# c-white/blacklight

Hardware: AMD Instinct MI355X
Metric: Mrays/sec + achieved HBM GB/s, 1024^2 camera over 256^3 GRMHD grid (higher is better)
Workload: dtype f64

## Files before the change

blacklight_amd/csrc/bl_geodesic.hip:

```cpp
#include "bl_kernel_util.h"
#include "bl_geodesic_common.h"
#include "bl_distance_closed.h"

namespace {

struct RayState {
  double y[8];
  double kt;
};

template <bool kWithDistance, bool kSpinZero>
__device__ __forceinline__ void rhs(const BlSpacetime &st, const double y[8], double kt, double k[8], double *r, int distance = BL_DISTANCE_EXACT) {
  double pos[3] = {y[1], y[2], y[3]};
  double kcov[4] = {kt, y[4], y[5], y[6]};
  double dpos[4], dk[3], ds = 0.0;
  bl_geodesic_rhs<kWithDistance, kSpinZero>(st, pos, kcov, dpos, dk, &ds, r, distance);
  k[0] = dpos[0];
  k[1] = dpos[1];
  k[2] = dpos[2];
  k[3] = dpos[3];
  k[4] = dk[0];
  k[5] = dk[1];
  k[6] = dk[2];
  k[7] = ds;
}

__device__ __forceinline__ long long traversal_to_ray(long long q, int res, const int *tile_order) {
  if (res <= 0) return q;
  int tiles_per_row = res >> 3;
  long long tile = tile_order != nullptr ? (long long)tile_order[q >> 6] : (q >> 6);
  int within = (int)(q & 63);
  long long tile_row = tile / tiles_per_row;
  int tile_col = (int)(tile % tiles_per_row);
  long long m2 = tile_row * 8 + (within >> 3);
  int m1 = tile_col * 8 + (within & 7);
  return m2 * res + m1;
}

__device__ __forceinline__ unsigned long long xcd_traversal(int r, long long j) {
  return (unsigned long long)(((j / BL_XCD_RUN) * BL_XCD_QUEUES + r) * BL_XCD_RUN + j % BL_XCD_RUN);
}
__device__ __forceinline__ long long xcd_queue_rays(int chunk_rays, int r) {
  const long long round = (long long)BL_XCD_RUN * BL_XCD_QUEUES;
  const long long full = chunk_rays / round, rest = chunk_rays - full * round - (long long)r * BL_XCD_RUN;
  return full * BL_XCD_RUN + (rest < 0 ? 0 : (rest < BL_XCD_RUN ? rest : BL_XCD_RUN));
}

}

template <bool kDormandPrince, bool kSpinZero>
__device__ __forceinline__ void bl_start_ray(const BlTraceArgs &P, const BlSpacetime &st, const BlCameraDevice &cam, long long pixel, long long ray, long long q) {
  double u_ind, v_ind, position[4], direction[4], factor;
  bl_pixel_indices(cam, pixel, P.block_locs, &u_ind, &v_ind);
  bl_pixel_ray(st, cam, u_ind, v_ind, position, direction, &factor);
  P.ray_constants[q] = make_double2(direction[0], factor);
  P.ray_out_index[q] = ray;
  if (P.camera_pos != nullptr)
    for (int mu = 0; mu < 4; mu++) P.camera_pos[4 * ray + mu] = position[mu];
  if (P.camera_dir != nullptr)
    for (int mu = 0; mu < 4; mu++) P.camera_dir[4 * ray + mu] = direction[mu];
  double *start = P.ray_start + q;
  const long long stride = P.ray_start_stride;
  RayState s;
  s.y[0] = position[0];
  s.y[1] = position[1];
  s.y[2] = position[2];
  s.y[3] = position[3];
  s.kt = direction[0];
  s.y[4] = direction[1];
  s.y[5] = direction[2];
  s.y[6] = direction[3];
  s.y[7] = 0.0;
  for (int p = 0; p < 7; p++) start[p * stride] = s.y[p];
  start[7 * stride] = s.kt;
  start[8 * stride] = bl_radial_coordinate<kSpinZero>(st, s.y[1], s.y[2], s.y[3]);
  if (kDormandPrince) {
    double k0[8], r_unused;
    rhs<true, kSpinZero>(st, s.y, s.kt, k0, &r_unused);
    for (int p = 0; p < 8; p++) start[(9 + p) * stride] = k0[p];
  }
}

template <bool kDormandPrince, bool kSpinZero>
__global__ void __launch_bounds__(256) bl_ray_init_kernel(BlTraceArgs P) {
  const long long q = (long long)blockIdx.x * blockDim.x + threadIdx.x;
  if (q >= (long long)P.chunk_rays) return;
  const BlSpacetime st = P.st;
  const long long ray = traversal_to_ray(P.chunk_begin + q, P.swizzle_tiles, P.tile_order);
  const long long pixel = P.pixel_map != nullptr ? (long long)P.pixel_map[ray] : ray;
  if (P.cameras == nullptr) {
    bl_start_ray<kDormandPrince, kSpinZero>(P, st, P.cam, pixel, ray, q);
    return;
  }
  const int camera = (int)(pixel / P.pixels_per_camera);
  const long long within = pixel - (long long)camera * P.pixels_per_camera;
  const int first = __builtin_amdgcn_readfirstlane(camera);
  if (__all(camera == first)) {
    const BlCameraDevice cam = P.cameras[first];
    bl_start_ray<kDormandPrince, kSpinZero>(P, st, cam, within, ray, q);
  } else {
    const BlCameraDevice cam = P.cameras[camera];
    bl_start_ray<kDormandPrince, kSpinZero>(P, st, cam, within, ray, q);
  }
}

#ifndef BL_GEO_WAVES
#define BL_GEO_WAVES 2
#endif
#ifndef BL_GEO_ONE_WAVE
#define BL_GEO_ONE_WAVE(integrator, with_time, spin_zero) ((integrator) == BL_INTEGRATOR_DP && ((with_time) || !(spin_zero)))
#endif
__device__ __forceinline__ int lane_here() {
  int l;
  asm volatile("v_mbcnt_lo_u32_b32 %0, -1, 0\n\tv_mbcnt_hi_u32_b32 %0, -1, %0" : "=v"(l));
  return l;
}
__device__ __forceinline__ int opaque_uniform(int v) {
  asm volatile("" : "+s"(v));
  return v;
}
__device__ __forceinline__ double opaque_uniform(double v) {
  asm volatile("" : "+s"(v));
  return v;
}
template <int kIntegrator, bool kTime, bool kSpinZero, bool kShell = false>
__global__ void __launch_bounds__(64, BL_GEO_ONE_WAVE(kIntegrator, kTime, kSpinZero) ? 1 : BL_GEO_WAVES) bl_geodesic_kernel(BlTraceArgs P) {
  const BlSpacetime st = P.st;

  bool have_ray = false;
  bool exhausted = false;
  RayState s;
  double k0[8];
  double h_new = 0.0, r_cur = 0.0, r_prev_sample = 0.0;
  int num_retry = 0, sample_num = 0, trunc_at = -1;
  int skipped = 0;
  int seg = 0;
  unsigned int slot = 0;
  bool previous_fail = false, flag = false;
  for (int p = 0; p < 8; p++) {
    s.y[p] = 0.0;
    k0[p] = 0.0;
  }
  s.kt = 0.0;
  long long block_next = 0, block_end = 0;
  constexpr bool kPark = kIntegrator == BL_INTEGRATOR_DP && !kTime && !kShell;
  __shared__ long long park_lds[5];
  typedef volatile __attribute__((address_space(3))) long long *ParkWord;
  const ParkWord park_word = (ParkWord)park_lds;
  if (kPark && lane_here() == 0) {
    park_lds[0] = reinterpret_cast<long long>(P.parked);
    park_lds[1] = (long long)P.park_capacity;
    const int below = (P.parked == nullptr || P.split_b_hi > 0.0) ? -1 : (P.park_always != 0 ? 64 : (P.park_below < 63 ? P.park_below : 63));
// ... 26 lines not shown
        const unsigned long long per_ray = (unsigned long long)P.ray_max_steps;
        const unsigned long long want = (unsigned long long)count * per_ray;
        const long long over = (long long)(atomicAdd(&P.counters[BL_CNT_COMMITTED], want) + want) - P.record_gate;
        long long refused = over > 0 ? (over + (long long)per_ray - 1) / (long long)per_ray : 0;
        refused = refused < (long long)count ? refused : (long long)count;
        admitted = count - (int)refused;
        long long give_back = -(refused * (long long)per_ray) + ((refused > 0 && over < kGateClosed / 2) ? kGateClosed : 0);
        if (admitted > 0 && P.xcd_state == nullptr) {
          base = atomicAdd(&P.counters[BL_CNT_NEXT_RAY], (unsigned long long)admitted);
          long long beyond = (long long)(base + (unsigned long long)admitted) - (long long)P.chunk_rays;
          beyond = beyond < 0 ? 0 : (beyond < (long long)admitted ? beyond : (long long)admitted);
          give_back -= beyond * (long long)per_ray;
        } else if (admitted > 0) {
          const int own = xcd_here();
          long long got = 0;
          for (int t = xcd_lds[0]; t < BL_XCD_QUEUES && got == 0; t++) {
            const int r = (own + t) & (BL_XCD_QUEUES - 1);
            const long long n_r = xcd_queue_rays(P.chunk_rays, r);
            const long long b = n_r > 0 ? (long long)atomicAdd(&P.xcd_state[r], (unsigned long long)admitted) : 0;
            if (b < n_r) {
              got = n_r - b < (long long)admitted ? n_r - b : (long long)admitted;
              base = (unsigned long long)b | ((unsigned long long)got << 40) | ((unsigned long long)r << 48);
            } else {
              xcd_lds[0] = t + 1;
            }
          }
          give_back -= ((long long)admitted - got) * (long long)per_ray;
        }
        if (give_back != 0) atomicAdd(&P.counters[BL_CNT_COMMITTED], (unsigned long long)give_back);
      }
      base = ((unsigned long long)(unsigned int)__builtin_amdgcn_readlane((int)(base >> 32), leader) << 32)
          | (unsigned long long)(unsigned int)__builtin_amdgcn_readlane((int)base, leader);
      admitted = __builtin_amdgcn_readlane(admitted, leader);
      if (need) {
        const int rank = __popcll(need_mask & ((1ull << lane) - 1ull));
        unsigned long long q = base + (unsigned long long)rank;
        bool wait = false;
        if (P.xcd_state != nullptr) {
          const int got = (int)((base >> 40) & 0xffull);
          q = xcd_traversal((int)(base >> 48), (long long)(base & 0xffffffffffull) + rank);
          wait = rank < admitted && rank >= got && got > 0;
          q = rank < got ? q : ~0ull;
        }
        if (wait) {
        } else if (rank >= admitted || q >= (unsigned long long)P.chunk_rays) {
          exhausted = true;
        } else {
          have_ray = true;
          slot = (unsigned int)q;
          const double *start = P.ray_start + q;
          const long long stride = P.ray_start_stride;
#pragma unroll
          for (int p = 0; p < 7; p++) s.y[p] = start[p * stride];
          s.y[7] = 0.0;
          s.kt = start[7 * stride];
          r_cur = start[8 * stride];
          if (kPark && r_cur < 0.0) {
            have_ray = false;
            atomicAdd(&P.counters[BL_CNT_COMMITTED], (unsigned long long)(-(long long)P.ray_max_steps));
          }
          if (kIntegrator == BL_INTEGRATOR_DP) {
#pragma unroll
            for (int p = 0; p < 8; p++) k0[p] = start[(9 + p) * stride];
          }
          h_new = -P.ray_step * r_cur;
          num_retry = 0;
          previous_fail = false;
          flag = false;
          sample_num = 0;
          skipped = 0;
          seg = 0;
          trunc_at = -1;
          r_prev_sample = 0.0;
        }
      }
    }
    if (kPark) {
      const long long word = park_word[2];
      const int park_below = __builtin_amdgcn_readfirstlane((int)word), park_after = __builtin_amdgcn_readfirstlane((int)(word >> 32));
      const unsigned long long holding = __ballot(have_ray);
      bool park = park_below >= 64;
      if (park_below >= 0 && !park) {
        const long long seen = park_word[3];
        int passes = __builtin_amdgcn_readfirstlane((int)seen);
        const int before = __builtin_amdgcn_readfirstlane((int)(seen >> 32));
        bool dry = passes > 0 || __ballot(exhausted) != 0ull;
        if (!dry && (before & 15) == 15)
          dry = __hip_atomic_load(&P.counters[BL_CNT_NEXT_RAY], __ATOMIC_RELAXED, __HIP_MEMORY_SCOPE_AGENT) >= (unsigned long long)P.chunk_rays;
        dry = __builtin_amdgcn_readfirstlane(dry ? 1 : 0) != 0;
        park_word[3] = dry ? (long long)(((unsigned long long)(unsigned int)before << 32) | (unsigned int)(passes + 1))
                           : (long long)((unsigned long long)(unsigned int)(before + 1) << 32);
        const int quiet = need_mask != 0ull ? 0 : __builtin_amdgcn_readfirstlane((int)park_word[4]) + 1;
        park_word[4] = (long long)quiet;
        park = dry && (__popcll(holding) <= park_below || passes >= park_after || quiet >= P.park_quiet);
      }
      if (park && holding != 0ull) {
        double *const parked = reinterpret_cast<double *>(park_word[0]);
        const long long park_capacity = park_word[1];
        const bool old_ray = have_ray && sample_num >= P.park_age;
        const unsigned long long old_mask = __ballot(old_ray), young_mask = holding & ~old_mask;
        const int leader = __ffsll((long long)holding) - 1;
        const int lane = lane_here();
        unsigned long long base_old = 0ull, base_young = 0ull;
        if (lane == leader) {
          if (old_mask != 0ull) base_old = atomicAdd(&P.counters[BL_CNT_PARKED], (unsigned long long)__popcll(old_mask));
          if (young_mask != 0ull) base_young = atomicAdd(&P.counters[BL_CNT_PARKED_YOUNG], (unsigned long long)__popcll(young_mask));
        }
        const int old_first = __builtin_amdgcn_readlane((int)base_old, leader), young_first = __builtin_amdgcn_readlane((int)base_young, leader);
        const unsigned long long below = (1ull << lane) - 1ull;
        const long long at = old_ray ? (long long)old_first + __popcll(old_mask & below)
                                     : park_capacity - 1 - ((long long)young_first + __popcll(young_mask & below));
        if (have_ray && at >= 0 && at < park_capacity) {
          double *pk = parked + at * BL_PARK_DOUBLES;
#pragma unroll
          for (int p = 0; p < 8; p++) {
            pk[p] = s.y[p];
            pk[8 + p] = k0[p];
          }
          pk[16] = s.kt;
          pk[17] = h_new;
          pk[18] = r_cur;
          pk[19] = r_prev_sample;
          pk[20] = __longlong_as_double((long long)(((unsigned long long)(unsigned int)sample_num << 32) | (unsigned long long)slot));
          pk[21] = __longlong_as_double((long long)(((unsigned long long)(unsigned int)trunc_at << 32) | (unsigned long long)(unsigned int)num_retry));
          pk[22] = __longlong_as_double((long long)(((unsigned long long)((previous_fail ? 1u : 0u) | (flag ? 2u : 0u)) << 32) | (unsigned long long)(unsigned int)seg));
          P.ray_offset[slot] = (long long)atomicAdd(&P.counters[BL_CNT_SAMPLES], (unsigned long long)P.ray_max_steps);
          have_ray = false;
        }
      }
    }
    if (__ballot(have_ray) == 0ull) {
      retire_record_slots(P.records_hot, P.record_stride, block_next, block_end, lane_here());
      break;
    }
#ifdef BL_GEO_STATS
    st_iter += 1;
    st_busy += have_ray ? 1 : 0;
    st_attempt += (have_ray && (kIntegrator != BL_INTEGRATOR_DP || num_retry <= P.ray_max_retries)) ? 1 : 0;
#endif

    int emit = 0;
    int num_steps = 0;
    int num_steps_ideal = 1;
    bool accepted = false;
    bool finish = false;
    double h = 0.0;
    double y5[8], k6[8], y4m[8];
    double rv0[8], rv1[8], rv2[8], rv3[8];
    double r_new = 0.0;
    for (int p = 0; p < 8; p++) {
      y5[p] = 0.0; k6[p] = 0.0; y4m[p] = 0.0; rv0[p] = 0.0; rv1[p] = 0.0; rv2[p] = 0.0; rv3[p] = 0.0;
    }

    if (have_ray) {
      if (kIntegrator == BL_INTEGRATOR_DP) {
        if (num_retry > P.ray_max_retries) {
          flag = true;
          finish = true;
        } else {
          h = h_new;
          double k1[8], k2[8], k3[8], k4[8], k5[8];
          double yt[8], r_stage;
          double t5 = s.y[0], t4 = s.y[0], s5 = s.y[7];
#ifdef BL_DISTANCE_FORCED
          const bool closed = BL_DISTANCE_FORCED != 0;
#else
          const bool closed = P.distance_mode != 0;
#endif
          double s_abs = 0.0, r_low = r_cur;
          if (closed) s5 = 0.0;
#define BL_FOLD(Q, K)                     \
          t5 += kB5[Q] * h * K[0];        \
          t4 += kB4[Q] * h * K[0];        \
          if (!closed) {                  \
            s5 += kB5[Q] * h * K[7];      \
          } else if (kB5[Q] != 0.0) {     \
            const double term = kB5[Q] * h * K[7]; \
            s5 += term;                   \
            s_abs += blm_abs(term);       \
          }
          BL_FOLD(0, k0)
#define BL_STAGE(S, KOUT, ...)                                                  \
          {                                                                      \
            const double *kq[6] = {__VA_ARGS__};                                 \
            _Pragma("unroll") for (int p = 1; p < 7; p++) {                      \
              double acc = s.y[p];                                               \
              _Pragma("unroll") for (int q = 0; q < S; q++) acc += kA[S][q] * h * kq[q][p]; \
              yt[p] = acc;                                                       \
            }                                                                    \
            yt[0] = 0.0; yt[7] = 0.0;                                            \
            rhs<true, kSpinZero>(st, yt, s.kt, KOUT, &r_stage, !closed ? BL_DISTANCE_EXACT : (S == 1 ? BL_DISTANCE_NONE : BL_DISTANCE_CLOSED)); \
            if (closed) r_low = std_min(r_low, r_stage);                         \
            BL_FOLD(S, KOUT)                                                     \
          }
          BL_STAGE(1, k1, k0, k0, k0, k0, k0, k0)
          BL_STAGE(2, k2, k0, k1, k0, k0, k0, k0)
          BL_STAGE(3, k3, k0, k1, k2, k0, k0, k0)
          BL_STAGE(4, k4, k0, k1, k2, k3, k0, k0)
          BL_STAGE(5, k5, k0, k1, k2, k3, k4, k0)
          BL_STAGE(6, k6, k0, k1, k2, k3, k4, k5)
#undef BL_STAGE
#undef BL_FOLD
          const double *kk[7] = {k0, k1, k2, k3, k4, k5, k6};
          double error = 0.0;
#pragma unroll
          for (int p = 0; p < 8; p++) {
            double a5 = s.y[p], a4 = s.y[p];
            if (p == 0 && !kTime) {
              a5 = t5;
              a4 = t4;
            } else if (p == 7) {
              a5 = closed ? (s.y[7] + s_abs) * kDistanceInflate : s5;
            } else {
#pragma unroll
              for (int q = 0; q < 7; q++) {
                a5 += kB5[q] * h * kk[q][p];
                a4 += kB4[q] * h * kk[q][p];
              }
            }
            y5[p] = a5;
            if (p < 7) {
              double y_abs = std_max(blm_abs(s.y[p]), blm_abs(a5));
              double error_scale = P.ray_tol_abs + P.ray_tol_rel * y_abs;
              double delta_y = blm_abs(a5 - a4);
              error = std_max(error, bl_div_g(delta_y, error_scale));
            }
          }
          r_new = r_stage;

          const double error_power = (error - error == 0.0 && error > 0.0) ? bl_pow_neg_fifth(error) : 0.0;
          if (!(error <= 1.0)) {
            double h_factor = 0.2;
            if (error - error == 0.0) {
              double h_factor_ideal = 0.9 * error_power;
              h_factor = std_max(h_factor_ideal, 0.2);
            }
            h_new = h * h_factor;
            num_retry += 1;
            previous_fail = true;
          } else {
            double h_factor = 10.0;
            if (error > 0.0) {
              h_factor = 0.9 * error_power;
              h_factor = std_max(h_factor, 0.2);
              h_factor = std_min(h_factor, 10.0);
            }
            if (previous_fail) h_factor = std_min(h_factor, 1.0);
            h_new = h * h_factor;
            num_retry = 0;
            previous_fail = false;
            accepted = true;

#pragma unroll
            for (int p = kTime ? 0 : 1; p < 7; p++) {
              double acc = s.y[p];
#pragma unroll
              for (int q = 0; q < 7; q++) acc += kB4m[q] * h * kk[q][p];
              y4m[p] = acc;
            }
            double r_mid = bl_radial_coordinate<kSpinZero>(st, y4m[1], y4m[2], y4m[3]);
            double delta_s_step = P.ray_step * r_mid;
            if (!closed) {
              double delta_s_full = y5[7] - s.y[7];
              num_steps_ideal = (int)ceil(delta_s_full / delta_s_step);
            } else {
              const BlRecip rc_step = bl_recip(delta_s_step);
              const double q_closed = bl_div_r(s5, rc_step);
              const double derived = kDistanceBandFactor * bl_div_r(bl_distance_bound_numerator(s_abs, y5[7]), rc_step);
              const double band = P.distance_mode == 2 ? std_max(derived, kDistanceWideBand) : derived;
              const double n_closed = ceil(q_closed);
              num_steps_ideal = (int)n_closed;
              if (!bl_distance_decided(q_closed, n_closed, band, st.ray_flat ? P.r_horizon : r_low, P.r_horizon)) atomicAdd(&P.counters[BL_CNT_UNDECIDED], 1ull);
            }
            int num_steps_max = P.ray_max_steps - sample_num;
            num_steps = num_steps_ideal;
            if (num_steps > num_steps_max) {
              num_steps = num_steps_max;
              flag = true;
            }
            emit = num_steps;
            if (num_steps_ideal > 1) {
#pragma unroll
              for (int p = kTime ? 0 : 1; p < 7; p++) {
                rv0[p] = y5[p] - s.y[p];
                rv1[p] = s.y[p] - y5[p] + h * k0[p];
                rv2[p] = 2.0 * (y5[p] - s.y[p]) - h * (k0[p] + k6[p]);
                double acc = 0.0;
#pragma unroll
                for (int q = 0; q < 7; q++) acc += kD[q] * h * kk[q][p];
                rv3[p] = acc;
              }
            } else {
#pragma unroll
              for (int p = kTime ? 0 : 1; p < 7; p++) {
                rv0[p] = -0.0; rv1[p] = -0.0; rv2[p] = -0.0; rv3[p] = -0.0;
              }
            }
          }
        }
      } else {
        double r = r_cur;
        h = -P.ray_step * (r - P.r_horizon);
        double kv[8], ysub[8], yacc[8], r_unused;
        if (kIntegrator == BL_INTEGRATOR_RK4) {
          rhs<false, kSpinZero>(st, s.y, s.kt, kv, &r_unused);
          for (int p = 0; p < 7; p++) yacc[p] = s.y[p] + 1.0 / 6.0 * h * kv[p];
          for (int p = 0; p < 7; p++) ysub[p] = s.y[p] + 0.5 * h * kv[p];
          ysub[7] = 0.0;
          rhs<false, kSpinZero>(st, ysub, s.kt, kv, &r_unused);
          for (int p = 0; p < 7; p++) yacc[p] += 1.0 / 3.0 * h * kv[p];
          for (int p = 0; p < 7; p++) ysub[p] = s.y[p] + 0.5 * h * kv[p];
          rhs<false, kSpinZero>(st, ysub, s.kt, kv, &r_unused);
          for (int p = 0; p < 7; p++) yacc[p] += 1.0 / 3.0 * h * kv[p];
          for (int p = 0; p < 7; p++) ysub[p] = s.y[p] + h * kv[p];
          rhs<false, kSpinZero>(st, ysub, s.kt, kv, &r_unused);
          for (int p = 0; p < 7; p++) yacc[p] += 1.0 / 6.0 * h * kv[p];
          for (int p = 0; p < 7; p++) y4m[p] = 0.5 * (s.y[p] + yacc[p]);
          for (int p = 0; p < 7; p++) y5[p] = yacc[p];
        } else {
          rhs<false, kSpinZero>(st, s.y, s.kt, kv, &r_unused);
          for (int p = 0; p < 7; p++) ysub[p] = s.y[p] + h * kv[p];
          ysub[7] = 0.0;
          for (int p = 0; p < 7; p++) yacc[p] = s.y[p] + 1.0 / 2.0 * h * kv[p];
          for (int p = 0; p < 7; p++) y4m[p] = yacc[p];
          rhs<false, kSpinZero>(st, ysub, s.kt, kv, &r_unused);
          for (int p = 0; p < 7; p++) y5[p] = yacc[p] + 1.0 / 2.0 * h * kv[p];
        }
        y5[7] = 0.0;
        for (int p = 0; p < 7; p++) {
          rv0[p] = -0.0; rv1[p] = -0.0; rv2[p] = -0.0; rv3[p] = -0.0;
        }
        accepted = true;
        num_steps_ideal = 1;
        num_steps = 1;
        emit = 1;
      }
    }

    if (kShell && emit > 0) {
      const bool dense = num_steps_ideal > 1;
      double d = 0.0, rr = 0.0;
#pragma unroll
      for (int p = 1; p < 4; p++) {
        const double b = dense ? s.y[p] : y4m[p];
        rr += b * b;
        d += (blm_abs(rv0[p]) + blm_abs(rv1[p])) + (blm_abs(rv2[p]) + blm_abs(rv3[p]));
      }
      const double low = P.skip_low + d, high = P.skip_high - d;
      if (rr > low * low && high > 0.0 && rr < high * high && trunc_at < 0) {
        skipped += emit;
        emit = 0;
        r_prev_sample = 0.0;
      }
    }

    const int scan = wave_inclusive_scan(emit);
    const int total = __builtin_amdgcn_readlane(scan, 63);
    const int excl = scan - emit;
    long long old_base = block_next, new_base = 0;
    int old_room = 0x7fffffff;
    if (total > 0) {
      const long long remaining = block_end - block_next;
      if ((long long)total <= remaining) {
        block_next += total;
      } else {
        old_room = (int)remaining;
        const unsigned long long grab = ((unsigned long long)std_max_ll((long long)total - remaining, BL_RECORD_BLOCK) + 63ull) & ~63ull;
        unsigned long long fetched = 0ull;
        if (lane_here() == 63) fetched = atomicAdd(&P.counters[BL_CNT_RECORDS], grab);
        fetched = ((unsigned long long)(unsigned int)__builtin_amdgcn_readlane((int)(fetched >> 32), 63) << 32)
            | (unsigned long long)(unsigned int)__builtin_amdgcn_readlane((int)fetched, 63);
        new_base = (long long)fetched;
        block_next = new_base + ((long long)total - remaining);
        block_end = (long long)(fetched + grab);
        if (P.xcd_lists != nullptr) {
          const int list = xcd_here();
          const unsigned int groups = (unsigned int)(grab >> 6);
          const int lane = lane_here();
          unsigned long long at = 0ull;
          if (lane == 0) at = atomicAdd(&P.xcd_state[BL_XCD_QUEUES + list], (unsigned long long)groups);
          at = ((unsigned long long)(unsigned int)__builtin_amdgcn_readfirstlane((int)(at >> 32)) << 32)
              | (unsigned long long)(unsigned int)__builtin_amdgcn_readfirstlane((int)at);
          for (unsigned int g = (unsigned int)lane; g < groups; g += 64u) {
            if (at + g < (unsigned long long)P.xcd_list_capacity) P.xcd_lists[(size_t)list * (size_t)P.xcd_list_capacity + at + g] = (unsigned int)(fetched >> 6) + g;
            else atomicExch(&P.counters[BL_CNT_OVERFLOW], 1ull);
          }
        }
        if (block_end > P.record_capacity) {
          atomicExch(&P.counters[BL_CNT_OVERFLOW], 1ull);
          block_end = block_next = 0;
          emit = 0;
        }
      }
    }

    const int max_emit = wave_max_nonneg(emit);
#ifdef BL_GEO_STATS
    st_emit_iter += max_emit;
    st_emit += emit;
    st_accept += accepted ? 1 : 0;
#endif
    const bool dense_output = num_steps_ideal > 1;
    double base[7];
#pragma unroll
    for (int p = kTime ? 0 : 1; p < 7; p++) base[p] = dense_output ? s.y[p] : y4m[p];
    const BlRecip rc_steps = bl_recip((double)num_steps_ideal);
    const double len = bl_div_r(h, rc_steps);
    double position = 0.5;
    for (int nn = 0; nn < max_emit; nn++, position += 1.0) {
      if (nn < emit) {
        double smp[7];
        const double frac = bl_div_r(position, rc_steps);
#pragma unroll
        for (int p = kTime ? 0 : 1; p < 7; p++)
          smp[p] = base[p] + frac * (rv0[p] + (1.0 - frac) * (rv1[p] + frac * (rv2[p] + (1.0 - frac) * rv3[p])));
        const int index = sample_num + nn;
        const double r_s = bl_radial_coordinate<kSpinZero>(st, smp[1], smp[2], smp[3]);
        const bool hit = index >= 1 && ((r_s > P.camera_r && r_s > r_prev_sample) || r_s < P.r_terminate);
        const bool dead = trunc_at >= 0 || hit;
        trunc_at = (trunc_at < 0 && hit) ? index : trunc_at;
        r_prev_sample = r_s;
        BlSampleHot hot;
        hot.x = smp[1];
        hot.y = smp[2];
        hot.z = smp[3];
        hot.ray = dead ? BL_DEAD_RAY : slot;
        hot.n = (unsigned int)(kShell ? index - skipped : index);
        const int place = excl + nn;
        const long long at = place < old_room ? old_base + place : new_base + (place - old_room);
        if (!kShell && P.segment_rows) {
          const bool first_of_group = nn == 0 || ((unsigned int)at & 15u) == 0u || place == old_room;
          seg += (!dead && first_of_group) ? 1 : 0;
          hot.n = (unsigned int)(seg - 1);
        }
        BlSampleCold cold;
        cold.kx = smp[4];
        cold.ky = smp[5];
        cold.kz = smp[6];
        cold.len = len;
        P.records_hot[at * P.record_stride] = hot;
        P.records_cold[at * P.record_stride] = cold;
        if (kTime) P.sample_t[at] = smp[0];
      }
    }

    if (have_ray && accepted) {
      double factor = bl_renormalization_factor<kSpinZero>(st, y5[1], y5[2], y5[3], s.kt, y5[4], y5[5], y5[6]);
      y5[4] *= factor;
      y5[5] *= factor;
      y5[6] *= factor;
      double r_before = r_cur;
      if (kIntegrator != BL_INTEGRATOR_DP) r_new = bl_radial_coordinate<kSpinZero>(st, y5[1], y5[2], y5[3]);
      sample_num += num_steps;
      bool terminate_outer = r_new > P.camera_r && r_new > r_before;
      bool terminate_inner = r_new < P.r_terminate;
      if (terminate_outer || terminate_inner) {
        finish = true;
      } else if (sample_num >= P.ray_max_steps) {
        flag = true;
        finish = true;
      }
#pragma unroll
      for (int p = 0; p < 8; p++) {
        s.y[p] = y5[p];
        k0[p] = k6[p];
      }
      r_cur = r_new;
    }
    if (have_ray && finish) {
      const int final_num = ((trunc_at >= 0) ? trunc_at : sample_num) - (kShell ? skipped : 0);
      P.ray_sample_num[slot] = final_num;
      if (kShell) P.ray_skipped[slot] = skipped;
      P.ray_flags[slot] = flag ? 1 : 0;
      const int rows = (!kShell && P.segment_rows) ? seg : final_num;
      if (!kShell && P.segment_rows) P.ray_rows[slot] = rows;
      P.ray_offset[slot] = (long long)atomicAdd(&P.counters[BL_CNT_SAMPLES], (unsigned long long)rows);
      atomicAdd(&P.counters[BL_CNT_COMMITTED], (unsigned long long)(-(long long)(P.ray_max_steps - (sample_num - (kShell ? skipped : 0)))));
      have_ray = false;
    }
  }
  if (P.xcd_state != nullptr) {
    __threadfence();
    const int lane = lane_here();
    unsigned long long ended = 0ull;
    if (lane == 0) ended = atomicAdd(&P.xcd_state[3 * BL_XCD_QUEUES], 1ull);
    ended = (unsigned long long)(unsigned int)__builtin_amdgcn_readfirstlane((int)ended);
    if (ended + 1ull == (unsigned long long)gridDim.x * (blockDim.x / 64u)) {
      long long first = P.chunk_rays;
      if (lane < BL_XCD_QUEUES) {
        const long long head = (long long)__hip_atomic_load(&P.xcd_state[lane], __ATOMIC_RELAXED, __HIP_MEMORY_SCOPE_AGENT);
        if (head < xcd_queue_rays(P.chunk_rays, lane)) first = (long long)xcd_traversal(lane, head);
      }
      long long done = P.chunk_rays;
      for (int r = 0; r < BL_XCD_QUEUES; r++) {
        const long long f = ((long long)(unsigned int)__builtin_amdgcn_readlane((int)(first >> 32), r) << 32)
            | (long long)(unsigned int)__builtin_amdgcn_readlane((int)first, r);
        done = f < done ? f : done;
      }
      if (lane == 0) atomicExch(&P.counters[BL_CNT_NEXT_RAY], (unsigned long long)done);
    }
  }
#ifdef BL_GEO_STATS
  atomicAdd(&P.counters[BL_CNT_DEBUG + 0], st_attempt);
  atomicAdd(&P.counters[BL_CNT_DEBUG + 1], st_accept);
  atomicAdd(&P.counters[BL_CNT_DEBUG + 2], st_emit);
  atomicAdd(&P.counters[BL_CNT_DEBUG + 6], st_busy);
  if (lane_here() == 0) {
    atomicAdd(&P.counters[BL_CNT_DEBUG + 3], st_iter);
    atomicAdd(&P.counters[BL_CNT_DEBUG + 4], st_emit_iter);
    atomicAdd(&P.counters[BL_CNT_DEBUG + 5], st_refill);
  }
#endif
}


__global__ void __launch_bounds__(256) bl_split_long_kernel(BlTraceArgs P) {
  const long long q = (long long)blockIdx.x * blockDim.x + threadIdx.x;
  if (q >= (long long)P.chunk_rays) return;
  const long long ray = P.ray_out_index[q];
  const long long pixel = P.pixel_map != nullptr ? (long long)P.pixel_map[ray] : ray;
  double u_ind, v_ind;
  bl_pixel_indices(P.cam, pixel, P.block_locs, &u_ind, &v_ind);
  const double scale = P.st.bh_m * P.cam.camera_width;
  const double b = blm_sqrt(u_ind * u_ind + v_ind * v_ind) * scale;
  if (!(b >= P.split_b_lo && b <= P.split_b_hi)) return;
  if (P.ray_start[q + 8 * P.ray_start_stride] < 0.0) return;
  const long long at = (long long)atomicAdd(&P.counters[BL_CNT_PARKED], 1ull);
  if (at >= (long long)P.park_capacity) return;
  double *start = P.ray_start + q;
  const long long stride = P.ray_start_stride;
  double *pk = P.parked + at * BL_PARK_DOUBLES;
  for (int p = 0; p < 7; p++) pk[p] = start[p * stride];
  pk[7] = 0.0;
  for (int p = 0; p < 8; p++) pk[8 + p] = start[(9 + p) * stride];
  const double r = start[8 * stride];
  pk[16] = start[7 * stride];
  pk[17] = -P.ray_step * r;
  pk[18] = r;
  pk[19] = 0.0;
  pk[20] = __longlong_as_double((long long)(unsigned long long)(unsigned int)q);
  pk[21] = __longlong_as_double((long long)(((unsigned long long)(unsigned int)-1) << 32));
  pk[22] = __longlong_as_double(0ll);
  pk[23] = 0.0;
  P.ray_offset[q] = (long long)atomicAdd(&P.counters[BL_CNT_SAMPLES], (unsigned long long)P.ray_max_steps);
  atomicAdd(&P.counters[BL_CNT_COMMITTED], (unsigned long long)P.ray_max_steps);
  start[8 * stride] = -r;
}

using BlTraceKernel = void (*)(BlTraceArgs);

extern "C" hipError_t bl_launch_split_long(const BlTraceArgs *args, hipStream_t stream) {
  if (args->parked == nullptr || args->ray_start == nullptr) return hipErrorInvalidValue;
  hipLaunchKernelGGL(bl_split_long_kernel, dim3((args->chunk_rays + 255) / 256), dim3(256), 0, stream, *args);
  return hipGetLastError();
}

extern "C" hipError_t bl_launch_ray_init(const BlTraceArgs *args, const KernelPlan::Geodesic &plan, hipStream_t stream) {
  const bool dp = plan.integrator == BL_INTEGRATOR_DP;
  if (plan.spin_zero && (!dp || args->st.bh_a != 0.0)) return hipErrorInvalidValue;
  BlTraceKernel kernel = plan.spin_zero ? bl_ray_init_kernel<true, true> : bl_ray_init_kernel<true, false>;
  hipLaunchKernelGGL(kernel, dim3((args->chunk_rays + 255) / 256), dim3(256), 0, stream, *args);
  return hipGetLastError();
}

template <int kIntegrator>
static BlTraceKernel fixed_step_kernel(const KernelPlan::Geodesic &g) {
  if (g.spin_zero || g.shell) return nullptr;
  return g.with_time ? bl_geodesic_kernel<kIntegrator, true, false, false> : bl_geodesic_kernel<kIntegrator, false, false, false>;
}
static BlTraceKernel geodesic_kernel(const KernelPlan::Geodesic &g) {
  constexpr int kDp = BL_INTEGRATOR_DP;
  if (g.integrator == BL_INTEGRATOR_RK4) return fixed_step_kernel<BL_INTEGRATOR_RK4>(g);
  if (g.integrator != kDp) return fixed_step_kernel<BL_INTEGRATOR_RK2>(g);
  if (g.with_time) return g.shell ? nullptr : (g.spin_zero ? bl_geodesic_kernel<kDp, true, true, false> : bl_geodesic_kernel<kDp, true, false, false>);
  if (g.spin_zero) return g.shell ? bl_geodesic_kernel<kDp, false, true, true> : bl_geodesic_kernel<kDp, false, true, false>;
  return g.shell ? bl_geodesic_kernel<kDp, false, false, true> : bl_geodesic_kernel<kDp, false, false, false>;
}

extern "C" hipError_t bl_launch_geodesic(const BlTraceArgs *args, const KernelPlan::Geodesic &plan, int grid, hipStream_t stream, int lds_pad) {
  BlTraceKernel kernel = geodesic_kernel(plan);
  if (kernel == nullptr || (args->sample_t != nullptr) != plan.with_time || (args->ray_skipped != nullptr) != plan.shell
      || (plan.spin_zero && args->st.bh_a != 0.0)) return hipErrorInvalidValue;
  hipLaunchKernelGGL(kernel, dim3(grid), dim3(64), lds_pad, stream, *args);
  return hipGetLastError();
}

extern "C" int bl_geodesic_occupancy(const KernelPlan::Geodesic &plan) {
  int blocks = 0;
  BlTraceKernel kernel = geodesic_kernel(plan);
  if (kernel == nullptr || hipOccupancyMaxActiveBlocksPerMultiprocessor(&blocks, kernel, 64, 0) != hipSuccess || blocks < 1) blocks = 4;
  return blocks;
}
```

blacklight_amd/csrc/bl_kernel_util.h:

```cpp
#pragma once
#include <hip/hip_runtime.h>

#include <cstddef>
#include <cstdlib>

#include "bl_device.h"
#include "bl_pol_frame.h"
#include "bl_bessel.h"

namespace {

constexpr double kPi = 3.141592653589793;
constexpr double kSqrt2 = 1.4142135623730951;
constexpr double kC = 2.99792458e10;
constexpr double kH = 6.62607015e-27;
constexpr double kMp = 1.67262192369e-24;
constexpr double kMe = 9.1093837015e-28;
constexpr double kE = 4.80320425e-10;
constexpr double kPow2_11_12 = 0x1.e3437e7101343p+0;
constexpr double kDeltaTauMax = 100.0;
constexpr long long kGateClosed = 1ll << 46;

__device__ __forceinline__ double std_max(double a, double b) { return (a < b) ? b : a; }
__device__ __forceinline__ double std_min(double a, double b) { return (b < a) ? b : a; }

__device__ __forceinline__ int wave_lane() { return threadIdx.x & 63; }


#define BL_DPP(old, src, ctrl, row_mask) __builtin_amdgcn_update_dpp((old), (src), (ctrl), (row_mask), 0xf, false)

__device__ __forceinline__ int wave_inclusive_scan(int v) {
  v += BL_DPP(0, v, 0x111, 0xf);
  v += BL_DPP(0, v, 0x112, 0xf);
  v += BL_DPP(0, v, 0x114, 0xf);
  v += BL_DPP(0, v, 0x118, 0xf);
  v += BL_DPP(0, v, 0x142, 0xa);
  v += BL_DPP(0, v, 0x143, 0xc);
  return v;
}

__device__ __forceinline__ int wave_max_nonneg(int v) {
  int t;
  t = BL_DPP(0, v, 0x111, 0xf); v = t > v ? t : v;
  t = BL_DPP(0, v, 0x112, 0xf); v = t > v ? t : v;
  t = BL_DPP(0, v, 0x114, 0xf); v = t > v ? t : v;
  t = BL_DPP(0, v, 0x118, 0xf); v = t > v ? t : v;
  t = BL_DPP(0, v, 0x142, 0xa); v = t > v ? t : v;
  t = BL_DPP(0, v, 0x143, 0xc); v = t > v ? t : v;
  return __builtin_amdgcn_readlane(v, 63);
}

__device__ __forceinline__ long long std_max_ll(long long a, long long b) { return a > b ? a : b; }

template <typename Args>
__device__ __forceinline__ const Args &kernel_arguments_in_place() {
#if defined(__HIP_DEVICE_COMPILE__)
  typedef const __attribute__((address_space(4))) Args *InSegment;
  InSegment p = (InSegment)__builtin_amdgcn_kernarg_segment_ptr();
  asm volatile("" : "+s"(p));
  return *(const Args *)p;
#else
  return *static_cast<const Args *>(nullptr);
#endif
}

__device__ __forceinline__ int xcd_here() {
#if defined(__HIP_DEVICE_COMPILE__)
  int x;
  asm volatile("s_getreg_b32 %0, hwreg(HW_REG_XCC_ID, 0, 4)" : "=s"(x));
  return x & 7;
#else
  return 0;
#endif
}

}
```

blacklight_amd/csrc/bl_shade_fused.hip:

```cpp
#include "bl_sampling_fast.h"

#pragma clang fp contract(fast)

#include "bl_local_angles.h"

#include <type_traits>

namespace fused2 {

struct alignas(16) AxisRow {
  double xf_lo, xf_hi;
  double xv;
  uint32_t dj_ge, dj_lt;
  double xv_ge, w_ge;
  double xv_lt, w_lt;
};
static_assert(sizeof(AxisRow) == 64, "axis row must be 64 bytes");

typedef const __attribute__((address_space(4))) BlShadeArgs *KernArgs;
__device__ __forceinline__ KernArgs kernargs() {
  KernArgs p = (KernArgs)__builtin_amdgcn_kernarg_segment_ptr();
  asm volatile("" : "+s"(p));
  return p;
}
// ... 869 lines not shown
  auto keep_geometry = [](Slot &s, const Geometry &g) __attribute__((always_inline)) {
    s.h0 = make_double2(g.hh, g.g_thth);
    s.h1.x = g.g_phph;
    s.c0 = make_double2(g.k_r, g.k_th);
    s.c1.x = -g.k_ph;
    s.loc.m_even = g.g_rr;
  };
  auto kept_geometry = [](const Slot &s) __attribute__((always_inline)) {
    Geometry g;
    g.hh = s.h0.x;
    g.g_thth = s.h0.y;
    g.g_phph = g.pp2 = s.h1.x;
    g.k_r = s.c0.x;
    g.k_th = s.c0.y;
    g.k_ph = s.c1.x;
    g.g_rr = s.loc.m_even;
    g.g_tph = g.g_rph = 0.0;
    return g;
  };
  Slot s0, s1, s2;
  s0.h0 = s0.c0 = s0.c1 = make_double2(0.0, 0.0);
  s0.h1 = make_double2(0.0, __longlong_as_double((long long)BL_DEAD_RAY));
  s0.kt = 0.0;
  s0.factor = 1.0;
  s0.row = 0;
  s0.loc.f_i = s0.loc.f_j = s0.loc.f_k = 0.0;
  s0.loc.status = kSampleNone;
  s0.loc.cell_bytes = 0u;
  s0.loc.m_even = 0.0;
  s0.loc.cell_ij = 0u;
  s0.loc.r_decided = false;
  s0.in = false;
  float4 lo[8], hi[8];
#pragma unroll
  for (int c = 0; c < 8; c++) lo[c] = hi[c] = make_float4(0.0f, 0.0f, 0.0f, 0.0f);
  s0.first = kNoRecords;
  s1.first = walk_next();
  s1.in = s1.first + lane_in_wave < n_records;
  {
    const double2 *rec = reinterpret_cast<const double2 *>(record_base(s1.first) + (size_t)(s1.in ? lane_bytes : 0u));
    s1.h0 = rec[0];
    s1.h1 = rec[1];
    s1.h1.y = s1.in ? s1.h1.y : __longlong_as_double((long long)BL_DEAD_RAY);
  }
  s1.loc = locate<kSpinZero, kRefined>(st, G, camera_r, band, (uint32_t)__double_as_longlong(s1.h1.y) != BL_DEAD_RAY, s1.h0.x, s1.h0.y, s1.h1.x, local_angles);
  uint32_t *deferred_here = reinterpret_cast<uint32_t *>(reinterpret_cast<char *>(lds) + (kRefined ? P.grid.fused_lds_bytes : 0)) + (kRefined ? (threadIdx.x >> 6) * 128u : 0u);
  uint32_t n_deferred_here = 0u;
  auto hand_over_deferred = [&](uint32_t first, uint32_t count) __attribute__((always_inline)) {
    KernArgs args = kernargs();
    const uint32_t lane = threadIdx.x & 63u;
    unsigned long long at = 0ull;
    if (lane == 0u) at = atomicAdd(&args->counters[BL_CNT_REDO], (unsigned long long)count);
    at = (unsigned long long)__builtin_amdgcn_readfirstlane((int)(at >> 32)) << 32 | (unsigned long long)(uint32_t)__builtin_amdgcn_readfirstlane((int)at);
    if (lane < count && at + lane < args->redo_capacity) args->redo_list[at + lane] = (unsigned long long)deferred_here[first + lane];
  };
  constexpr int kWalkPlain = 0, kWalkMirrorNext = 1, kWalkPlainNext = 2;
  auto iteration = [&](Slot &p, Slot &c, Slot &x, auto kLocal, auto kWalkIs) __attribute__((always_inline)) {
    constexpr int kWalk = decltype(kWalkIs)::value;
    constexpr bool kMirrorNext = kWalk == kWalkMirrorNext, kMirrorCur = kWalk == kWalkPlainNext, kMirrorPrev = kWalk == kWalkMirrorNext;
    const uint32_t ray = (uint32_t)__double_as_longlong(p.h1.y);
    const bool live = ray != BL_DEAD_RAY;
    const uint32_t n = (uint32_t)(((unsigned long long)__double_as_longlong(p.h1.y)) >> 32);
    const uint32_t status = p.loc.status & 0xffu;
    const bool interp = status == (uint32_t)kSampleInterp;
    if constexpr (kMirrorNext) {
      x.first = c.first < n_records ? c.first + n_records : c.first;
      x.in = c.in;
      x.h1.y = c.h1.y;
    } else {
      x.first = walk_next();
      x.in = x.first + lane_in_wave < n_records;
      const double2 *rec = reinterpret_cast<const double2 *>(record_base(x.first) + (size_t)(x.in ? lane_bytes : 0u));
      x.h0 = rec[0];
      x.h1 = rec[1];
    }
    const double kt = p.kt, momentum_factor = p.factor;
    const long long row_first = kMirrorPrev ? p.row + (long long)P.row_add : p.row;
    float pr[8];
    const bool near_midpoint = trilinear(lo, hi, p.loc.f_i, p.loc.f_j, p.loc.f_k, pr);
    if (kFactors) {
#pragma unroll
      for (int q = 0; q < 8; q++) asm volatile("" : "+v"(pr[q]));
    }
    gathers_wave += (unsigned long long)__popcll(__ballot(interp));
    fused2::gather_issue(cells, c.loc.cell_bytes, (c.loc.status & 0xffu) == (uint32_t)kSampleInterp, row_bytes, plane_bytes, lo, hi);
    if constexpr (kMirrorCur) {
      c.c1.y = p.c1.y;
      c.kt = p.kt;
      c.factor = p.factor;
      c.row = p.row;
    } else {
      const double2 *rec = reinterpret_cast<const double2 *>(record_base(c.first) + (size_t)(c.in ? lane_bytes : 0u));
      c.c0 = rec[2];
      c.c1 = rec[3];
      const uint32_t ray_cur = (uint32_t)__double_as_longlong(c.h1.y);
      const uint32_t ray_slot = ray_cur != BL_DEAD_RAY ? ray_cur : 0u;
      const double2 constants = bl_ray_constants(ray_constants, (size_t)ray_slot);
      c.kt = constants.x;
      c.factor = constants.y;
      c.row = *reinterpret_cast<const long long *>(ray_offset + (size_t)(ray_slot << 3));
    }
    bool have = false, undecided_cut = false;
    double2 rec = make_double2(1.0, 0.0);
    double2 factors[4];
    if (kFactors) factors[0] = factors[1] = factors[2] = factors[3] = make_double2(0.0, 0.0);
    if (interp) {
      if constexpr (kWalk != kWalkPlain) {
        Geometry geometry;
        if constexpr (kMirrorPrev) {
          geometry = kept_geometry(p);
        } else {
          geometry = shade_geometry<kSpinZero>(st, p.h0.x, p.h0.y, p.h1.x, p.c0.x, p.c0.y, p.c1.x, kt);
          keep_geometry(c, geometry);
        }
        rec = shade_plasma<kSpinZero, kFactors>(K, freq, freq_inv, x_unit, cut_mask, cut_table, pr, geometry, kt, momentum_factor, -p.c1.y, &have, &undecided_cut);
      } else {
        rec = shade<kSpinZero, kFactors>(st, K, freq, freq_inv, x_unit, cut_mask, cut_table, pr, p.h0.x, p.h0.y, p.h1.x, p.c0.x, p.c0.y, p.c1.x, kt, momentum_factor,
                                         -p.c1.y, &have, &undecided_cut, kFactors ? &factors : nullptr, kFactors && model_rows,
                                         kFactors ? P.n_sigma_bands : 0, P.sigma_band_lo, P.sigma_band_hi);
      }
    }
    const bool defer = interp && (undecided_cut || near_midpoint || (p.loc.status & kPlainUndecided) != 0u);
    if (!(interp && have)) rec = make_double2(1.0, (status == (uint32_t)kSampleOffGrid && fallback_nan) ? nan : 0.0);
    if (kFactors) {
      if (live && !defer) {
        if (!interp) factors[0].x = (status == (uint32_t)kSampleOffGrid && fallback_nan) ? 2.0 : 0.0;
        double2 *out = reinterpret_cast<double2 *>(P.freq_inputs + (size_t)(row_first + (long long)n));
        out[0] = factors[0];
        out[1] = factors[1];
        out[2] = factors[2];
        out[3] = factors[3];
      }
    } else if (!kComposed) {
      if (live && !defer) {
        double2 *out = P.transfer + (size_t)(row_first + (long long)n);
        *out = rec;
      }
    } else {
      const uint32_t key_lo = ray, key_hi = n;
      const uint32_t below_lo = (uint32_t)BL_DPP((int)~key_lo, (int)key_lo, 0x111, 0xf), below_hi = (uint32_t)BL_DPP((int)key_hi, (int)key_hi, 0x111, 0xf);
      const unsigned long long first = __ballot(below_lo != key_lo || below_hi != key_hi) | 0x0001000100010001ull;
      const unsigned long long needs_records = __ballot(live && (defer || BL_IS_AFFINE_THICK(rec.x)));
      bool expand = false;
      if (__builtin_expect(needs_records != 0ull, 0)) {
        unsigned long long m = needs_records;
        m |= m >> 1; m |= m >> 2; m |= m >> 4; m |= m >> 8;
        expand = __builtin_amdgcn_inverse_ballot_w64((m & 0x0001000100010001ull) * 0xffffull);
      }
      if (!expand) {
        const unsigned long long g2 = first | (first << 1), g4 = g2 | (g2 << 2), g8 = g4 | (g4 << 4);
        double a = rec.x, c = rec.y;
#define BL_COMPOSE_STEP(CTRL, STARTS)                                                                                          \
        {                                                                                                                      \
          const double a_below = __hiloint2double(BL_DPP(0, __double2hiint(a), CTRL, 0xf), BL_DPP(0, __double2loint(a), CTRL, 0xf)); \
          const double c_below = __hiloint2double(BL_DPP(0, __double2hiint(c), CTRL, 0xf), BL_DPP(0, __double2loint(c), CTRL, 0xf)); \
          if (__builtin_amdgcn_inverse_ballot_w64(~(STARTS))) {                                                                \
            c = __builtin_fma(a_below, c, c_below);                                                                            \
            a = a_below * a;                                                                                                   \
          }                                                                                                                    \
        }
        BL_COMPOSE_STEP(0x111, first)
        BL_COMPOSE_STEP(0x112, g2)
        BL_COMPOSE_STEP(0x114, g4)
        BL_COMPOSE_STEP(0x118, g8)
#undef BL_COMPOSE_STEP
        const unsigned long long last_lanes = (first >> 1) | 0x8000800080008000ull;
        if (__builtin_amdgcn_inverse_ballot_w64(last_lanes) && live) P.composed[(size_t)(row_first + (long long)n)] = make_double2(a, c);
      } else {
        const uint32_t record = p.first + lane_in_wave;
        if (live && !defer) P.transfer[record] = rec;
        const unsigned long long last_lanes = (first >> 1) | 0x8000800080008000ull;
        const uint32_t lane = threadIdx.x & 63u;
        if (((last_lanes >> lane) & 1ull) != 0ull && live) {
          const unsigned long long starts_below = first & ((2ull << lane) - 1ull);
          const uint32_t length = lane - (63u - (uint32_t)__builtin_clzll(starts_below)) + 1u;
          P.composed[(size_t)(row_first + (long long)n)] =
              make_double2(-(double)length, __longlong_as_double((long long)(unsigned long long)(record - (length - 1u))));
        }
      }
    }
    if (kRefined) {
      const unsigned long long waiting = __ballot(live && defer);
      if (__builtin_expect(waiting != 0ull, 0)) {
        const uint32_t lane = threadIdx.x & 63u;
        if (live && defer) deferred_here[n_deferred_here + (uint32_t)__popcll(waiting & ((1ull << lane) - 1ull))] = p.first + lane_in_wave;
        n_deferred_here += (uint32_t)__popcll(waiting);
        if (n_deferred_here >= 64u) {
          n_deferred_here -= 64u;
          hand_over_deferred(n_deferred_here, 64u);
        }
      }
    } else if (__builtin_expect(live && defer, 0)) {
      KernArgs args = kernargs();
      unsigned long long *counters = args->counters;
      const unsigned long long at = atomicAdd(&counters[BL_CNT_REDO], 1ull);
      if (at < args->redo_capacity) args->redo_list[at] = (unsigned long long)(p.first + lane_in_wave);
    }
    constexpr int kAngles = decltype(kLocal)::value ? kAnglesLocal : kAnglesGlobal;
    if constexpr (kMirrorNext)
      x.loc = locate_mirror<kAngles>(st, G, band, c.loc, c.h0.x, -c.h0.y);
    else
      x.loc = locate<kSpinZero, kRefined, kAngles>(st, G, camera_r, band, x.in && (uint32_t)__double_as_longlong(x.h1.y) != BL_DEAD_RAY, x.h0.x, x.h0.y, x.h1.x, local_angles);
    x.h1.y = x.in ? x.h1.y : __longlong_as_double((long long)BL_DEAD_RAY);
  };
  auto loop = [&](auto kLocal, auto kPaired) __attribute__((always_inline)) {
    constexpr int kFirst = decltype(kPaired)::value ? kWalkMirrorNext : kWalkPlain, kSecond = decltype(kPaired)::value ? kWalkPlainNext : kWalkPlain;
    const std::integral_constant<int, kFirst> first;
    const std::integral_constant<int, kSecond> second;
    for (;;) {
      if (!__any(s0.in || s1.in)) break;
      iteration(s0, s1, s2, kLocal, first);
      if (!__any(s1.in || s2.in)) break;
      iteration(s1, s2, s0, kLocal, second);
      if (!__any(s2.in || s0.in)) break;
      iteration(s2, s0, s1, kLocal, first);
      if constexpr (decltype(kPaired)::value) {
        if (!__any(s0.in || s1.in)) break;
        iteration(s0, s1, s2, kLocal, second);
        if (!__any(s1.in || s2.in)) break;
        iteration(s1, s2, s0, kLocal, first);
        if (!__any(s2.in || s0.in)) break;
        iteration(s2, s0, s1, kLocal, second);
      }
    }
  };
  auto walk = [&](auto kLocal) __attribute__((always_inline)) {
    if constexpr (kPairs) {
      if (P.row_add != 0u) {
        loop(kLocal, std::true_type{});
        return;
      }
    }
    loop(kLocal, std::false_type{});
  };
#if defined(BLV_ANGLES)
  walk(std::integral_constant<bool, !kRefined && BLV_ANGLES == 1>{});
#else
  if (!kRefined && local_angles) walk(std::integral_constant<bool, !kRefined>{});
  else walk(std::false_type{});
#endif
  if (kRefined && n_deferred_here != 0u) hand_over_deferred(0u, n_deferred_here);
  if ((threadIdx.x & 63) == 0 && gathers_wave != 0ull) atomicAdd(&P.counters[BL_CNT_GATHERS], gathers_wave);
}
#pragma clang fp contract(off)

namespace fused2 {

struct LocatedExact {
  double f_i, f_j, f_k, ph_unwrapped;
  uint32_t status, cell_bytes;
};

__device__ __forceinline__ bool guess_confirmed(uint32_t table, int guess, double s) {
  const v2d faces = lds_read2(table + ((uint32_t)guess << 6));
  return s <= faces.y && (guess == 0 || s > faces.x);
}
__device__ __forceinline__ void axis_lookup_exact(uint32_t table, int cell, double s, double *frac, uint32_t *anchor) {
  const uint32_t row_addr = table + ((uint32_t)cell << 6);
  const v4u mid = lds_read_bits(row_addr + 16u);
  const bool ge = s >= __hiloint2double((int)mid.y, (int)mid.x);
  const v2d centre = lds_read2(row_addr + (ge ? 32u : 48u));
  *anchor = (uint32_t)cell - (ge ? mid.z : mid.w);
  *frac = blm_div(s - centre.x, centre.y);
}

template <bool kSpinZero, bool kMeshes = false>
__device__ __forceinline__ LocatedExact locate_exact(const BlSpacetime &st, const BlGridDevice &g, const GridScalars &G, double camera_r, bool live, double x1, double x2,
                                                     double x3) {
  x1 = live ? x1 : 1.0;
  x2 = live ? x2 : 1.0;
  x3 = live ? x3 : 1.0;
  double r2;
  const double r = bl_radial_coordinate2<kSpinZero>(st, x1, x2, x3, &r2);
  const bool cut = r > camera_r;
  const double th = bl_acos(blm_div(x3, r));
  const double ph_unwrapped = kSpinZero ? bl_atan2(x2, x1) : bl_atan2(x2, x1) - bl_atan(blm_div(st.bh_a, r));
  double ph = ph_unwrapped;
  ph += ph < 0.0 ? 2.0 * kPi : 0.0;
  ph -= ph >= 2.0 * kPi ? 2.0 * kPi : 0.0;
  const bool off_grid = r < G.r_in || r > G.r_out;
  const bool sampled = live && !cut && !off_grid;
  if (kMeshes && G.lds_desc != 0u) {
    KernArgs A = kernargs();
    const int n_box_i1 = A->grid.n_edge[0] - 1, n_box_j1 = A->grid.n_edge[1] - 1, n_box_k1 = A->grid.n_edge[2] - 1;
    const uint32_t n_box_i = (uint32_t)A->grid.n_edge[0], n_box_j = (uint32_t)A->grid.n_edge[1];
    const float log2_r = __builtin_amdgcn_logf((float)r);
    int bi = (int)((log2_r - A->grid.box_l0) * A->grid.box_linv);
    int bj = (int)((th - A->grid.box_x0[0]) * A->grid.box_inv_w[0]);
    int bk = (int)((ph - A->grid.box_x0[1]) * A->grid.box_inv_w[1]);
    bi = bi < 0 ? 0 : (bi > n_box_i1 ? n_box_i1 : bi);
    bj = bj < 0 ? 0 : (bj > n_box_j1 ? n_box_j1 : bj);
    bk = bk < 0 ? 0 : (bk > n_box_k1 ? n_box_k1 : bk);
    v4u desc = lds_read_bits(G.lds_desc + ((__umul24(__umul24((uint32_t)bk, n_box_j) + (uint32_t)bj, n_box_i) + (uint32_t)bi) << 4));
    const v4u head_r = lds_read_bits(desc.y);
    const v2d head_th = lds_read2(desc.z), head_ph = lds_read2(desc.w);
    int ci = (int)((log2_r - __uint_as_float(head_r.x)) * __uint_as_float(head_r.y));
    int cj = (int)((th - head_th.x) * head_th.y);
    int ck = (int)((ph - head_ph.x) * head_ph.y);
    ci = ci < 0 ? 0 : (ci > G.n_i1 ? G.n_i1 : ci);
    cj = cj < 0 ? 0 : (cj > G.n_j1 ? G.n_j1 : cj);
    ck = ck < 0 ? 0 : (ck > G.n_k1 ? G.n_k1 : ck);
    auto faces_of = [&](uint32_t rows, int c) { return lds_read2(rows + 16u + ((uint32_t)c << 6)); };
    auto inside = [&](uint32_t rows, int c, double x) {
      const v2d faces = faces_of(rows, c);
      return x > faces.x && x <= faces.y;
    };
    if (__builtin_expect(sampled && !(inside(desc.y, ci, r) && inside(desc.z, cj, th) && inside(desc.w, ck, ph)), 0)) {
      for (int step = 0; step < 3 * 4096; step++) {
// ... 376 lines not shown
```

Before: 34.03.

## Flatten DP give-up branch, strength-reduce record addressing, use bound_ctrl DPP shifts

Hoists the retry-exhausted check for the Dormand-Prince integrator out of the main step branch so the give-up path skips the stage setup. Replaces the per-sample record index select and multiply with a running byte offset that switches once at the old/new region boundary. Switches the row-shift DPP ops in the wave scan, wave max and compose steps to bound_ctrl zero-fill, which may let the compiler drop the old-value move. These are small instruction-count cuts in hot loops; they change correctness assumptions only if the byte offset or the 32-bit slot index overflows.

```diff
diff --git a/blacklight_amd/csrc/bl_geodesic.hip b/blacklight_amd/csrc/bl_geodesic.hip
--- a/blacklight_amd/csrc/bl_geodesic.hip
+++ b/blacklight_amd/csrc/bl_geodesic.hip
@@ -1,3 +1,5 @@
+#include <type_traits>
+
 #include "bl_kernel_util.h"
 #include "bl_geodesic_common.h"
 #include "bl_distance_closed.h"
@@ -330,9 +332,15 @@
       y5[p] = 0.0; k6[p] = 0.0; y4m[p] = 0.0; rv0[p] = 0.0; rv1[p] = 0.0; rv2[p] = 0.0; rv3[p] = 0.0;
     }
 
-    if (have_ray) {
+    constexpr bool kFlatGiveUp = kIntegrator == BL_INTEGRATOR_DP && !BL_GEO_ONE_WAVE(kIntegrator, kTime, kSpinZero);
+    const bool gave_up = kFlatGiveUp && have_ray && num_retry > P.ray_max_retries;
+    if (gave_up) {
+      flag = true;
+      finish = true;
+    }
+    if (have_ray && !gave_up) {
       if (kIntegrator == BL_INTEGRATOR_DP) {
-        if (num_retry > P.ray_max_retries) {
+        if (!kFlatGiveUp && num_retry > P.ray_max_retries) {
           flag = true;
           finish = true;
         } else {
@@ -585,6 +593,13 @@
     const BlRecip rc_steps = bl_recip((double)num_steps_ideal);
     const double len = bl_div_r(h, rc_steps);
     double position = 0.5;
+    static_assert(sizeof(BlSampleHot) == sizeof(BlSampleCold), "one running offset serves both record arrays");
+    const long long record_bytes = (long long)P.record_stride * (long long)sizeof(BlSampleHot);
+    const long long new_offset = new_base * record_bytes;
+    const long long first_slot = excl < old_room ? old_base + excl : new_base + (excl - old_room);
+    using RecordSlot = typename std::conditional<kTime, long long, unsigned int>::type;
+    RecordSlot at = (RecordSlot)first_slot;
+    long long at_offset = first_slot * record_bytes;
     for (int nn = 0; nn < max_emit; nn++, position += 1.0) {
       if (nn < emit) {
         double smp[7];
@@ -605,7 +620,10 @@
         hot.ray = dead ? BL_DEAD_RAY : slot;
         hot.n = (unsigned int)(kShell ? index - skipped : index);
         const int place = excl + nn;
-        const long long at = place < old_room ? old_base + place : new_base + (place - old_room);
+        if (__builtin_expect(place == old_room, 0)) {
+          at = (RecordSlot)new_base;
+          at_offset = new_offset;
+        }
         if (!kShell && P.segment_rows) {
           const bool first_of_group = nn == 0 || ((unsigned int)at & 15u) == 0u || place == old_room;
           seg += (!dead && first_of_group) ? 1 : 0;
@@ -616,9 +634,11 @@
         cold.ky = smp[5];
         cold.kz = smp[6];
         cold.len = len;
-        P.records_hot[at * P.record_stride] = hot;
-        P.records_cold[at * P.record_stride] = cold;
+        *reinterpret_cast<BlSampleHot *>(reinterpret_cast<char *>(P.records_hot) + at_offset) = hot;
+        *reinterpret_cast<BlSampleCold *>(reinterpret_cast<char *>(P.records_cold) + at_offset) = cold;
         if (kTime) P.sample_t[at] = smp[0];
+        at += 1;
+        at_offset += record_bytes;
       }
     }
 
diff --git a/blacklight_amd/csrc/bl_kernel_util.h b/blacklight_amd/csrc/bl_kernel_util.h
--- a/blacklight_amd/csrc/bl_kernel_util.h
+++ b/blacklight_amd/csrc/bl_kernel_util.h
@@ -28,12 +28,13 @@
 
 
 #define BL_DPP(old, src, ctrl, row_mask) __builtin_amdgcn_update_dpp((old), (src), (ctrl), (row_mask), 0xf, false)
+#define BL_DPP_ZERO(src, ctrl) __builtin_amdgcn_update_dpp(0, (src), (ctrl), 0xf, 0xf, true)
 
 __device__ __forceinline__ int wave_inclusive_scan(int v) {
-  v += BL_DPP(0, v, 0x111, 0xf);
-  v += BL_DPP(0, v, 0x112, 0xf);
-  v += BL_DPP(0, v, 0x114, 0xf);
-  v += BL_DPP(0, v, 0x118, 0xf);
+  v += BL_DPP_ZERO(v, 0x111);
+  v += BL_DPP_ZERO(v, 0x112);
+  v += BL_DPP_ZERO(v, 0x114);
+  v += BL_DPP_ZERO(v, 0x118);
   v += BL_DPP(0, v, 0x142, 0xa);
   v += BL_DPP(0, v, 0x143, 0xc);
   return v;
@@ -41,10 +42,10 @@
 
 __device__ __forceinline__ int wave_max_nonneg(int v) {
   int t;
-  t = BL_DPP(0, v, 0x111, 0xf); v = t > v ? t : v;
-  t = BL_DPP(0, v, 0x112, 0xf); v = t > v ? t : v;
-  t = BL_DPP(0, v, 0x114, 0xf); v = t > v ? t : v;
-  t = BL_DPP(0, v, 0x118, 0xf); v = t > v ? t : v;
+  t = BL_DPP_ZERO(v, 0x111); v = t > v ? t : v;
+  t = BL_DPP_ZERO(v, 0x112); v = t > v ? t : v;
+  t = BL_DPP_ZERO(v, 0x114); v = t > v ? t : v;
+  t = BL_DPP_ZERO(v, 0x118); v = t > v ? t : v;
   t = BL_DPP(0, v, 0x142, 0xa); v = t > v ? t : v;
   t = BL_DPP(0, v, 0x143, 0xc); v = t > v ? t : v;
   return __builtin_amdgcn_readlane(v, 63);
diff --git a/blacklight_amd/csrc/bl_shade_fused.hip b/blacklight_amd/csrc/bl_shade_fused.hip
--- a/blacklight_amd/csrc/bl_shade_fused.hip
+++ b/blacklight_amd/csrc/bl_shade_fused.hip
@@ -1045,8 +1045,8 @@
         double a = rec.x, c = rec.y;
 #define BL_COMPOSE_STEP(CTRL, STARTS)                                                                                          \
         {                                                                                                                      \
-          const double a_below = __hiloint2double(BL_DPP(0, __double2hiint(a), CTRL, 0xf), BL_DPP(0, __double2loint(a), CTRL, 0xf)); \
-          const double c_below = __hiloint2double(BL_DPP(0, __double2hiint(c), CTRL, 0xf), BL_DPP(0, __double2loint(c), CTRL, 0xf)); \
+          const double a_below = __hiloint2double(BL_DPP_ZERO(__double2hiint(a), CTRL), BL_DPP_ZERO(__double2loint(a), CTRL)); \
+          const double c_below = __hiloint2double(BL_DPP_ZERO(__double2hiint(c), CTRL), BL_DPP_ZERO(__double2loint(c), CTRL)); \
           if (__builtin_amdgcn_inverse_ballot_w64(~(STARTS))) {                                                                \
             c = __builtin_fma(a_below, c, c_below);                                                                            \
             a = a_below * a;                                                                                                   \
```

After: 34.17 (median of 6 runs). About the same (+0.4%).
